# lipku/LiveTalking

Hardware: NVIDIA H100
Metric: lip-sync frames/sec (wav2lip256, 256x256, batch 16, mel + U-Net fwd + paste-back) (higher is better)
Workload: dtype f16 (fp32 accumulate); mel f64; paste u8

## Files before the change

### livetalking_b200/csrc/conv_gather.cu

```cuda
#include "conv_params.h"
#include "ltb_internal.h"
#include "ptx_sm90.cuh"

namespace ltb {

constexpr int kGatherThreads = 256;

template <int BN, int KB>
struct GatherCfg {
  static constexpr int CH = KB / 8;
  static constexpr int ROWB = KB * 2;
  static constexpr int RSTEP = kGatherThreads / CH;
  static constexpr int RPT = 128 / RSTEP;
  static constexpr int A_BYTES = 128 * ROWB;
  static constexpr int B_BYTES = (BN * ROWB < 1024) ? 1024 : BN * ROWB;
  static constexpr int STAGE_BYTES = A_BYTES + B_BYTES;
  static constexpr int STAGES = (STAGE_BYTES >= 32768) ? 3 : 4;
  static constexpr uint32_t LAYOUT = (KB == 64) ? 1u : (KB == 32) ? 2u : 3u;
  static constexpr uint32_t SBO = 8 * ROWB;
  static constexpr int SMEM_BYTES = STAGES * STAGE_BYTES + 1024;
};

template <int KB>
__device__ __forceinline__ uint32_t swz_chunk(int row, int j) {
  if (KB == 64) return (uint32_t)(j ^ (row & 7));
  if (KB == 32) return (uint32_t)(j ^ ((row >> 1) & 3));
  return (uint32_t)(j ^ ((row >> 2) & 1));
}

template <int BN, int KB, bool GRP>
__global__ void __launch_bounds__(kGatherThreads) conv_gather_wgmma_kernel(const __grid_constant__ ConvParams p) {
  using C = GatherCfg<BN, KB>;
  extern __shared__ uint8_t smem_raw[];
  const int tid = threadIdx.x;
  const int wg = tid >> 7, wq = (tid >> 5) & 3, lane = tid & 31;
  const uint32_t tiles = (smem_u32(smem_raw) + 1023u) & ~1023u;

  const int zphase = (p.ksplit > 1) ? 0 : ((p.zbatch > 1) ? (int)(blockIdx.z % p.nphases) : (int)blockIdx.z);
  const ConvPhase& ph = p.ph[zphase];
  const __half* in_base = p.in;
  const __half* w_base = p.w;
  __half* out_base = p.out;
  if (p.zbatch > 1) {
    const int zb = blockIdx.z / p.nphases;
    const int zo = zb / p.zdiv, zi = zb - zo * p.zdiv;
    in_base += zo * p.in_zo + zi * p.in_zi;
    w_base += zo * p.w_zo + zi * p.w_zi;
    out_base += zo * p.out_zo + zi * p.out_zi;
  }
  const int g_rows = GRP ? p.group_images * p.GH * p.GW : 0, g_tiles = (g_rows + 127) / 128;
  const int group = GRP ? (int)blockIdx.x / g_tiles : 0;
  const int m0 = GRP ? group * g_rows + ((int)blockIdx.x - group * g_tiles) * 128 : blockIdx.x * 128;
  const int n0 = blockIdx.y * BN;
  const int cpt = p.Cin / KB;
  int it_begin = 0, kiters = ph.ntaps * cpt;
  if (p.ksplit > 1) {
    const int per = (kiters + p.ksplit - 1) / p.ksplit;
    it_begin = (int)blockIdx.z * per;
    kiters = min(per, kiters - it_begin);
  }
  pdl_launch_dependents();
  pdl_wait();
  const float* bias_g = nullptr;
  if constexpr (GRP) {
    const int slot = p.group_slot[group];
    w_base += slot * p.w_slot_stride;
    bias_g = p.bias + slot * p.bias_slot_stride;
  }
  const float* const bias = GRP ? bias_g : p.bias;
  const int M = GRP ? (group + 1) * g_rows : p.M;

  const int j = tid % C::CH;
  const int r0 = tid / C::CH;
  int riy[C::RPT], rix[C::RPT];
  long long rbase[C::RPT];
  const int gsz = p.GH * p.GW;
#pragma unroll
  for (int i = 0; i < C::RPT; ++i) {
    const int m = m0 + r0 + i * C::RSTEP;
    if (m < M) {
      const int b = m / gsz;
      const int rem = m - b * gsz;
      const int gy = rem / p.GW;
      const int gx = rem - gy * p.GW;
      riy[i] = gy * p.sy;
      rix[i] = gx * p.sx;
      rbase[i] = ((long long)(b * p.IH + riy[i]) * p.IW + rix[i]) * p.ICtot + p.ic_off + j * 8;
    } else {
      riy[i] = -(1 << 20);
      rix[i] = 0;
      rbase[i] = 0;
    }
  }
  auto load = [&](int it) {
    const int kk = it_begin + it;
    const int tap = kk / cpt, cc = kk - tap * cpt;
    const uint32_t a_base = tiles + (it % C::STAGES) * C::STAGE_BYTES;
    const uint32_t b_base = a_base + C::A_BYTES;
    const int dy = ph.dy[tap], dx = ph.dx[tap];
    const long long toff = (long long)(dy * p.IW + dx) * p.ICtot + cc * KB;
#pragma unroll
    for (int i = 0; i < C::RPT; ++i) {
      const int row = r0 + i * C::RSTEP;
      const int iy = riy[i] + dy, ix = rix[i] + dx;
      const bool inb = ((unsigned)iy < (unsigned)p.IH) && ((unsigned)ix < (unsigned)p.IW);
      const __half* src = inb ? (in_base + rbase[i] + toff) : in_base;
      cp_async16(a_base + row * C::ROWB + swz_chunk<KB>(row, j) * 16, src, inb ? 16u : 0u);
    }
    const size_t wk = (size_t)ph.koff + (size_t)tap * p.Cin + cc * KB + j * 8;
#pragma unroll
    for (int i = 0; i < C::RPT; ++i) {
      const int n = r0 + i * C::RSTEP;
      if (n < BN) cp_async16(b_base + n * C::ROWB + swz_chunk<KB>(n, j) * 16, w_base + (size_t)(n0 + n) * p.Ktot + wk, 16u);
    }
  };

  float acc[BN / 2];
#pragma unroll
  for (int i = 0; i < BN / 2; ++i) acc[i] = 0.f;
#pragma unroll
  for (int s = 0; s < C::STAGES - 1; ++s) {
    if (s < kiters) load(s);
    cp_async_commit();
  }
  for (int it = 0; it < kiters; ++it) {
    cp_async_wait<C::STAGES - 2>();
    fence_proxy_async_smem();
    __syncthreads();
    if (it + C::STAGES - 1 < kiters) load(it + C::STAGES - 1);
    cp_async_commit();
    const uint32_t a_base = tiles + (it % C::STAGES) * C::STAGE_BYTES;
    const uint32_t b_base = a_base + C::A_BYTES;
    wgmma_fence();
#pragma unroll
    for (int k = 0; k < KB / 16; ++k) {
      const uint64_t ad = wgmma_desc(a_base + wg * 64 * C::ROWB + k * 32, 16, C::SBO, C::LAYOUT);
      const uint64_t bd = wgmma_desc(b_base + k * 32, 16, C::SBO, C::LAYOUT);
      Wgmma<BN>::ss(acc, ad, bd, 1u);
    }
    wgmma_commit();
    wgmma_wait<0>();
    wgmma_fence_regs(acc);
  }
  cp_async_wait<0>();

  const int cq = 2 * (lane & 3);
#pragma unroll
  for (int hh = 0; hh < 2; ++hh) {
    const int m = m0 + wg * 64 + wq * 16 + (lane >> 2) + 8 * hh;
    if (m >= M) continue;
    if (p.ksplit > 1) {
      float* wrow = p.ws + ((size_t)blockIdx.z * p.M + m) * p.Cout + n0;
#pragma unroll
      for (int i = 0; i < BN / 8; ++i)
        *reinterpret_cast<float2*>(wrow + 8 * i + cq) = make_float2(acc[4 * i + 2 * hh], acc[4 * i + 2 * hh + 1]);
      continue;
    }
    const int b = m / gsz;
    const int rem = m - b * gsz;
    const int gy = rem / p.GW;
    const int gx = rem - gy * p.GW;
    const size_t opix = (size_t)(b * p.OH + gy * p.osy + ph.ooy) * p.OW + gx * p.osx + ph.oox;
    __half* optr = out_base + opix * p.OCtot + p.oc_off + n0;
    const __half* rptr = p.res ? (p.res + opix * p.RCtot + p.rc_off + n0) : nullptr;
#pragma unroll
    for (int i = 0; i < BN / 8; ++i) {
      const int c = 8 * i + cq;
      const float2 bb = __ldg(reinterpret_cast<const float2*>(bias + n0 + c));
      float x = acc[4 * i + 2 * hh] + bb.x, y = acc[4 * i + 2 * hh + 1] + bb.y;
      if (rptr) {
        const float2 rf = __half22float2(__ldcg(reinterpret_cast<const __half2*>(rptr + c)));
        x += rf.x;
        y += rf.y;
      }
      if (p.relu) {
        x = fmaxf(x, 0.f);
        y = fmaxf(y, 0.f);
      }
      x = fminf(fmaxf(x, -65504.f), 65504.f);
      y = fminf(fmaxf(y, -65504.f), 65504.f);
      *reinterpret_cast<__half2*>(optr + c) = __floats2half2_rn(x, y);
    }
  }
}

template <int BN, int KB, bool GRP>
static cudaError_t launch_grp(const ConvParams& p, cudaStream_t st) {
  using C = GatherCfg<BN, KB>;
  static SmemConfigOnce once;
  if (cudaError_t e = once.ensure(conv_gather_wgmma_kernel<BN, KB, GRP>, C::SMEM_BYTES); e != cudaSuccess) return e;
  const int mt = GRP ? (p.N / p.group_images) * ((p.group_images * p.GH * p.GW + 127) / 128) : (p.M + 127) / 128;
  dim3 grid(mt, p.Cout / BN, p.ksplit > 1 ? p.ksplit : p.nphases * (p.zbatch > 1 ? p.zbatch : 1));
  return launch_kernel_pdl(conv_gather_wgmma_kernel<BN, KB, GRP>, grid, dim3(kGatherThreads), C::SMEM_BYTES, st, p);
}

template <int BN, int KB>
static cudaError_t launch_one(const ConvParams& p, cudaStream_t st) {
  return p.group_slot ? launch_grp<BN, KB, true>(p, st) : launch_grp<BN, KB, false>(p, st);
}

template <int KB>
static cudaError_t launch_kb(const ConvParams& p, int bn, cudaStream_t st) {
  switch (bn) {
    case 128: return launch_one<128, KB>(p, st);
    case 64: return launch_one<64, KB>(p, st);
    case 32: return launch_one<32, KB>(p, st);
    case 16: return launch_one<16, KB>(p, st);
  }
  return cudaErrorInvalidValue;
}

static int conv_gather_pick_bn(const ConvParams& p) {
  int bn = 0;
  for (int c : {128, 64, 32, 16})
    if (p.Cout % c == 0) {
      bn = c;
      break;
    }
  if (!bn) return 0;
  const long mt = (p.M + 127) / 128;
  const long zb = p.zbatch > 1 ? p.zbatch : 1;
  while (bn > 32 && mt * (p.Cout / bn) * p.nphases * zb < 132) bn >>= 1;
  return bn;
}

__global__ void __launch_bounds__(256) splitk_finalize_kernel(const float* __restrict__ ws, int ksplit, int M, int Cout,
                                                              const float* __restrict__ bias, const __half* __restrict__ res, int RCtot,
                                                              int rc_off, int relu, __half* __restrict__ out, int OCtot, int oc_off) {
  const unsigned vpr = Cout / 8;
  const unsigned total = (unsigned)M * vpr;
  const size_t slice = (size_t)M * Cout;
  pdl_launch_dependents();
  pdl_wait();
  for (unsigned i = blockIdx.x * 256u + threadIdx.x; i < total; i += gridDim.x * 256u) {
    const size_t m = i / vpr;
    const int c = (int)(i % vpr) * 8;
    float f[8];
#pragma unroll
    for (int j = 0; j < 8; ++j) f[j] = __ldg(bias + c + j);
    for (int s = 0; s < ksplit; ++s) {
      const float4* w4 = reinterpret_cast<const float4*>(ws + s * slice + m * Cout + c);
      const float4 a = __ldcg(w4), b = __ldcg(w4 + 1);
      f[0] += a.x; f[1] += a.y; f[2] += a.z; f[3] += a.w;
      f[4] += b.x; f[5] += b.y; f[6] += b.z; f[7] += b.w;
    }
    if (res) {
      const uint4 rv = __ldcg(reinterpret_cast<const uint4*>(res + m * RCtot + rc_off + c));
      const __half* rh = reinterpret_cast<const __half*>(&rv);
#pragma unroll
      for (int j = 0; j < 8; ++j) f[j] += __half2float(rh[j]);
    }
    uint4 ov;
    __half* oh = reinterpret_cast<__half*>(&ov);
#pragma unroll
    for (int j = 0; j < 8; ++j) {
      float x = relu ? fmaxf(f[j], 0.f) : f[j];
      oh[j] = __float2half_rn(fminf(fmaxf(x, -65504.f), 65504.f));
    }
    *reinterpret_cast<uint4*>(out + m * OCtot + oc_off + c) = ov;
  }
}

bool conv_gather_pick(const ConvParams& p, bool have_ws, size_t splitk_ws_floats, int* bn_out, int* kb_out, int* ksplit_out) {
  if (p.Cout % 16 != 0 || p.Cin % 16 != 0 || (p.ICtot % 8) || (p.OCtot % 8) || (p.ic_off % 8) || (p.oc_off % 8) ||
      (p.Ktot % 8) || p.nphases < 1 || p.nphases > kMaxPhases)
    return false;
  if (p.res && ((p.RCtot % 8) || (p.rc_off % 8))) return false;
  int bn = conv_gather_pick_bn(p);
  if (!bn) return false;
  const int kb = (p.Cin % 64 == 0) ? 64 : (p.Cin % 32 == 0) ? 32 : 16;
  int ksplit = 0;
  const int kiters = p.ph[0].ntaps * (p.Cin / kb);
  const long mt = (p.M + 127) / 128;
  if (have_ws && !p.group_slot && p.nphases == 1 && p.zbatch <= 1 && p.osy == 1 && p.osx == 1 && p.GH == p.OH && p.GW == p.OW && kiters >= 32 && mt <= 8) {
    int bn2 = 0;
    for (int c : {128, 64, 32, 16})
      if (p.Cout % c == 0) {
        bn2 = c;
        break;
      }
    const long tiles = mt * (p.Cout / bn2);
    if (tiles < 64) {
      int ks = (int)((264 + tiles - 1) / tiles);
      if (ks > kiters / 8) ks = kiters / 8;
      if (ks > 32) ks = 32;
      while (ks >= 2 && (size_t)ks * p.M * p.Cout > splitk_ws_floats) --ks;
      if (ks >= 2) {
        const int per = (kiters + ks - 1) / ks;
        ksplit = (kiters + per - 1) / per;
        bn = bn2;
      }
    }
  }
  *bn_out = bn;
  *kb_out = kb;
  *ksplit_out = ksplit;
  return true;
}

cudaError_t launch_conv_gather(const ConvParams& p_in, cudaStream_t st, float* splitk_ws, size_t splitk_ws_floats) {
  ConvParams p = p_in;
  int bn, kb;
  if (!conv_gather_pick(p, splitk_ws != nullptr, splitk_ws_floats, &bn, &kb, &p.ksplit)) return cudaErrorInvalidValue;
  p.ws = p.ksplit > 1 ? splitk_ws : nullptr;
  cudaError_t e;
  if (kb == 64) e = launch_kb<64>(p, bn, st);
  else if (kb == 32) e = launch_kb<32>(p, bn, st);
  else e = launch_kb<16>(p, bn, st);
  if (e != cudaSuccess || p.ksplit <= 1) return e;
  const size_t total = (size_t)p.M * (p.Cout / 8);
  int blocks = (int)((total + 255) / 256);
  if (blocks > 592) blocks = 592;
  return launch_kernel_pdl(splitk_finalize_kernel, dim3(blocks), dim3(256), 0, st, (const float*)p.ws, p.ksplit, p.M, p.Cout, p.bias, p.res,
                           p.RCtot, p.rc_off, p.relu, p.out, p.OCtot, p.oc_off);
}

}
```

### livetalking_b200/csrc/conv_plan.cu

```cuda
#include <cstring>
#include <string>
#include <vector>

#include "../../include/ltb200.h"
#include "conv_plan.h"
#include "ltb_internal.h"

namespace ltb {

static const int kTd[2][2] = {{0, 0}, {0, 1}};
static const int kTk[2][2] = {{1, 0}, {2, 0}};
static const int kTn[2] = {1, 2};
static const int kUd[2][2] = {{-1, 0}, {0, 1}};

ConvParams conv_params(ConvMode mode, int N, ConvSlice in, int IH, int IW, int Cin, ConvSlice out, int OH, int OW, int Cout,
                       ConvSlice res, const __half* w, int Ktot, int w_koff, const float* bias, bool relu, ConvTaps taps) {
  ConvParams p;
  std::memset(&p, 0, sizeof(p));
  p.in = in.p;
  p.N = N;
  p.IH = IH;
  p.IW = IW;
  p.ICtot = in.Ctot;
  p.ic_off = in.off;
  p.Cin = Cin;
  p.sy = p.sx = 1;
  p.out = const_cast<__half*>(out.p);
  p.OH = OH;
  p.OW = OW;
  p.OCtot = out.Ctot;
  p.oc_off = out.off;
  p.osy = p.osx = 1;
  p.Cout = Cout;
  p.res = res.p;
  p.RCtot = res.Ctot;
  p.rc_off = res.off;
  p.w = w;
  p.Ktot = Ktot;
  p.bias = bias;
  p.relu = relu ? 1 : 0;
  if (mode == ConvMode::Dense) {
    p.sy = taps.sy;
    p.sx = taps.sx;
    p.GH = OH;
    p.GW = OW;
    p.nphases = 1;
    ConvPhase& ph = p.ph[0];
    ph.ntaps = taps.KH * taps.KW;
    ph.koff = w_koff;
    for (int kh = 0; kh < taps.KH; ++kh)
      for (int kw = 0; kw < taps.KW; ++kw) {
        ph.dy[kh * taps.KW + kw] = (signed char)(kh - taps.pad_t);
        ph.dx[kh * taps.KW + kw] = (signed char)(kw - taps.pad_l);
      }
  } else {
    const bool up = mode == ConvMode::Upsample2x;
    p.GH = IH;
    p.GW = IW;
    p.osy = p.osx = 2;
    p.nphases = 4;
    p.upconv = up ? 1 : 0;
    int koff = w_koff;
    for (int a = 0; a < 2; ++a)
      for (int b = 0; b < 2; ++b) {
        ConvPhase& ph = p.ph[a * 2 + b];
        const int na = up ? 2 : kTn[a], nb = up ? 2 : kTn[b];
        ph.ntaps = na * nb;
        ph.koff = koff;
        ph.ooy = a;
        ph.oox = b;
        for (int i = 0; i < na; ++i)
          for (int j = 0; j < nb; ++j) {
            ph.dy[i * nb + j] = (signed char)(up ? kUd[a][i] : kTd[a][i]);
            ph.dx[i * nb + j] = (signed char)(up ? kUd[b][j] : kTd[b][j]);
          }
        koff += ph.ntaps * Cin;
      }
  }
  p.M = N * p.GH * p.GW;
  return p;
}

int conv_plan(const ConvParams& p, const __half* w_tap, ConvPath path, ConvPlan* out) {
  out->p = p;
  out->halo = false;
  if (p.group_slot) {
    if (p.group_images < 1 || p.N % p.group_images || p.slots < 1 || p.w_slot_stride < 0 || p.bias_slot_stride < 0)
      return LTB_FAIL("conv: grouped weights need N divisible by group_images >= 1, slots >= 1 and non-negative slot strides");
    if (p.zbatch > 1 || p.upconv) return LTB_FAIL("conv: grouped weights cannot be combined with zbatch or the fused upsample");
  }
  if (path == ConvPath::Gather) return 0;
  const bool gemm = p.nphases == 1 && p.ph[0].ntaps == 1;
  if (!((w_tap || gemm) && conv_halo_supported(p))) {
    if (path == ConvPath::Auto) return 0;
    return LTB_FAIL("conv: the halo kernel cannot run " + std::to_string(p.N) + "x" + std::to_string(p.IH) + "x" + std::to_string(p.IW) +
                    "x" + std::to_string(p.Cin) + " -> " + std::to_string(p.OH) + "x" + std::to_string(p.OW) + "x" + std::to_string(p.Cout) +
                    (w_tap || gemm ? "" : " without tap-major weights"));
  }
  if (conv_halo_make_plan(p, w_tap, &out->hp) != 0) return LTB_FAIL("conv: halo plan / tensor map creation failed");
  out->halo = true;
  return 0;
}

cudaError_t conv_launch(const ConvPlan& pl, cudaStream_t st, float* splitk_ws, size_t ws_floats) {
  return pl.halo ? launch_conv_halo(pl.hp, st) : launch_conv_gather(pl.p, st, splitk_ws, ws_floats);
}

bool conv_plan_variant(const ConvPlan& pl, bool have_ws, size_t ws_floats, ltb_conv_variant* out) {
  std::memset(out, 0, sizeof(*out));
  out->grouped = pl.p.group_slot != nullptr;
  if (pl.halo) {
    out->kernel = 1;
    out->taps = pl.hp.TAPS;
    out->bn = pl.hp.BN;
    out->nsub = pl.hp.NSUB;
    out->nacc = pl.hp.NACC;
    out->resident_chunks = conv_halo_resident_chunks(pl.hp, conv_halo_sms());
    out->res_halo = pl.hp.hp.res_halo;
    return true;
  }
  int ksplit = 0;
  if (!conv_gather_pick(pl.p, have_ws, ws_floats, &out->bn, &out->kb, &ksplit)) return false;
  out->ksplit = ksplit > 1 ? ksplit : 1;
  return true;
}

bool conv_plan_fuse_gn_stats(ConvPlan* pl, float* stats, int groups, int hw) {
  const ConvParams& p = pl->p;
  if (!pl->halo || pl->hp.grouped || p.oc_off != 0 || p.OCtot != p.Cout || !conv_halo_gn_fusable(pl->hp, p.Cout, groups, hw)) return false;
  HaloParams& h = pl->hp.hp;
  h.gn_stats = stats;
  h.gn_groups = groups;
  h.gn_cpg = p.Cout / groups;
  h.gn_hw = hw;
  h.gn_images = p.M / hw;
  return true;
}

bool conv_plan_fuse_head(ConvPlan* pl, const float* w, const float* b, float* out) {
  if (!pl->halo || pl->hp.grouped || pl->hp.BN != 32 || pl->p.Cout != 32) return false;
  pl->hp.hp.head_w = w;
  pl->hp.hp.head_b = b;
  pl->hp.hp.head_out = out;
  return true;
}

static void pack_conv_w(const float* w, int cout, int cin, int KH, int KW, std::vector<__half>& out) {
  out.resize((size_t)cout * KH * KW * cin);
  for (int co = 0; co < cout; ++co)
    for (int kh = 0; kh < KH; ++kh)
      for (int kw = 0; kw < KW; ++kw)
        for (int ci = 0; ci < cin; ++ci)
          out[((size_t)co * KH * KW + kh * KW + kw) * cin + ci] = __float2half(w[(((size_t)co * cin + ci) * KH + kh) * KW + kw]);
}
static void pack_convT_w(const float* w, int cin, int cout, std::vector<__half>& out) {
  out.resize((size_t)cout * 9 * cin);
  for (int co = 0; co < cout; ++co) {
    size_t k = 0;
    for (int a = 0; a < 2; ++a)
      for (int b = 0; b < 2; ++b)
        for (int i = 0; i < kTn[a]; ++i)
          for (int j = 0; j < kTn[b]; ++j) {
            const int kh = kTk[a][i], kw = kTk[b][j];
            for (int ci = 0; ci < cin; ++ci, ++k)
              out[(size_t)co * 9 * cin + k] = __float2half(w[(((size_t)ci * cout + co) * 3 + kh) * 3 + kw]);
          }
  }
}

}

using namespace ltb;

static int conv2d_f16_impl(const ltb_conv_desc* d, const void* in_f16, const float* w_f32, const float* bias_f32,
                           const void* res_f16, void* out_f16, int reps, float* ms_out) {
  if (!d || !in_f16 || !w_f32 || !bias_f32 || !out_f16) return LTB_FAIL("null argument");
  if (d->has_res && !res_f16) return LTB_FAIL("has_res set but res is null");
  int OH, OW, Ktot;
  std::vector<__half> wp;
  if (d->transposed) {
    if (d->KH != 3 || d->KW != 3) return LTB_FAIL("transposed conv: only k=3,s=2,p=1,op=1");
    OH = d->IH * 2;
    OW = d->IW * 2;
    Ktot = 9 * d->Cin;
    pack_convT_w(w_f32, d->Cin, d->Cout, wp);
  } else {
    if (d->KH * d->KW > kMaxTaps) return LTB_FAIL("kernel too large");
    OH = conv_out_dim(d->IH, d->KH, d->sy, d->pad);
    OW = conv_out_dim(d->IW, d->KW, d->sx, d->pad);
    Ktot = d->KH * d->KW * d->Cin;
    pack_conv_w(w_f32, d->Cout, d->Cin, d->KH, d->KW, wp);
  }
  if (OH <= 0 || OW <= 0) return LTB_FAIL("empty output");
  const size_t in_b = (size_t)d->N * d->IH * d->IW * d->Cin * 2, out_b = (size_t)d->N * OH * OW * d->Cout * 2;
  __half *din = nullptr, *dout = nullptr, *dw = nullptr, *dres = nullptr, *dwt = nullptr;
  float* dbias = nullptr;
  float* dws = nullptr;
  cudaEvent_t e0 = nullptr, e1 = nullptr;
  int rc = 0;
  auto cleanup = [&]() {
    cudaFree(din);
    cudaFree(dout);
    cudaFree(dw);
    cudaFree(dres);
    cudaFree(dwt);
    cudaFree(dws);
    cudaFree(dbias);
    if (e0) cudaEventDestroy(e0);
    if (e1) cudaEventDestroy(e1);
  };
#define CK(x)                                                             \
  do {                                                                    \
    cudaError_t _e = (x);                                                 \
    if (_e != cudaSuccess) {                                              \
      rc = LTB_FAIL(std::string(#x) + ": " + cudaGetErrorString(_e));     \
      cleanup();                                                          \
      return rc;                                                          \
    }                                                                     \
  } while (0)
  CK(cudaMalloc(&din, in_b));
  CK(cudaMalloc(&dout, out_b));
  CK(cudaMalloc(&dw, wp.size() * 2));
  CK(cudaMalloc(&dbias, (size_t)d->Cout * 4));
  CK(cudaMemcpy(din, in_f16, in_b, cudaMemcpyHostToDevice));
  CK(cudaMemcpy(dw, wp.data(), wp.size() * 2, cudaMemcpyHostToDevice));
  CK(cudaMemcpy(dbias, bias_f32, (size_t)d->Cout * 4, cudaMemcpyHostToDevice));
  CK(cudaMemset(dout, 0xFF, out_b));
  if (d->has_res) {
    CK(cudaMalloc(&dres, out_b));
    CK(cudaMemcpy(dres, res_f16, out_b, cudaMemcpyHostToDevice));
  }
  if (d->KH == 3 && d->KW == 3) {
    CK(cudaMalloc(&dwt, wp.size() * 2));
    CK(d->transposed ? launch_w_tap_major_convT(dw, dwt, d->Cout, d->Cin, nullptr) : launch_w_tap_major(dw, dwt, d->Cout, d->Cin, nullptr));
  }
  const ConvParams p = conv_params(d->transposed ? ConvMode::Transposed : ConvMode::Dense, d->N, {din, d->Cin, 0}, d->IH, d->IW, d->Cin,
                                   {dout, d->Cout, 0}, OH, OW, d->Cout, d->has_res ? ConvSlice{dres, d->Cout, 0} : ConvSlice{}, dw, Ktot, 0,
                                   dbias, d->relu != 0, {d->KH, d->KW, d->sy, d->sx, d->pad, d->pad});
  const ConvPath path = d->force_path == 1 ? ConvPath::Gather : d->force_path == 2 ? ConvPath::Halo : ConvPath::Auto;
  ConvPlan pl;
  if (conv_plan(p, dwt, path, &pl)) {
    cleanup();
    return 1;
  }
  const size_t ws_floats = pl.halo ? 0 : (size_t)1 << 22;
  if (ws_floats) {
    CK(cudaMalloc(&dws, ws_floats * sizeof(float)));
    CK(cudaMemset(dws, 0, ws_floats * sizeof(float)));
  }
  CK(conv_launch(pl, nullptr, dws, ws_floats));
  if (reps > 0) {
    CK(cudaEventCreate(&e0));
    CK(cudaEventCreate(&e1));
    for (int i = 0; i < 3; ++i) CK(conv_launch(pl, nullptr, dws, ws_floats));
    CK(cudaEventRecord(e0, nullptr));
    for (int i = 0; i < reps; ++i) CK(conv_launch(pl, nullptr, dws, ws_floats));
    CK(cudaEventRecord(e1, nullptr));
    CK(cudaEventSynchronize(e1));
    CK(cudaEventElapsedTime(ms_out, e0, e1));
    *ms_out /= reps;
  }
  CK(cudaDeviceSynchronize());
  CK(cudaMemcpy(out_f16, dout, out_b, cudaMemcpyDeviceToHost));
#undef CK
  cleanup();
  return 0;
}

extern "C" {

int ltb_conv2d_f16(const ltb_conv_desc* d, const void* in_f16, const float* w_f32, const float* bias_f32,
                   const void* res_f16, void* out_f16) {
  return conv2d_f16_impl(d, in_f16, w_f32, bias_f32, res_f16, out_f16, 0, nullptr);
}

int ltb_conv2d_f16_timed(const ltb_conv_desc* d, const void* in_f16, const float* w_f32, const float* bias_f32,
                         const void* res_f16, void* out_f16, int reps, float* ms_per_launch) {
  if (reps < 1 || !ms_per_launch) return LTB_FAIL("conv2d_f16_timed: reps >= 1 and a result pointer are required");
  return conv2d_f16_impl(d, in_f16, w_f32, bias_f32, res_f16, out_f16, reps, ms_per_launch);
}

}
```

Baseline: 6889.

## Extend split-K to transposed-conv phases and 1x1 row GEMMs; route small convs to gather

Generalizes the split-K gather path so the grid z-dimension covers phases times k-splits, letting the 4-phase transposed convolutions and tiny 1x1 spatial GEMMs split their reduction across more CTAs. The finalize kernel now takes the full params and maps each phase's rows back to strided output pixels for residual and output writes. Small-spatial 3x3 and transposed convs (<=4x4) skip the halo kernel and use the gather/split-K path by default. This targets under-filled SMs on the low-resolution U-Net layers, at the cost of an fp32 workspace round trip and an extra finalize launch.

```diff
diff --git a/livetalking_b200/csrc/conv_gather.cu b/livetalking_b200/csrc/conv_gather.cu
--- a/livetalking_b200/csrc/conv_gather.cu
+++ b/livetalking_b200/csrc/conv_gather.cu
@@ -1,3 +1,5 @@
+#include <algorithm>
+
 #include "conv_params.h"
 #include "ltb_internal.h"
 #include "ptx_sm90.cuh"
@@ -36,7 +38,7 @@
   const int wg = tid >> 7, wq = (tid >> 5) & 3, lane = tid & 31;
   const uint32_t tiles = (smem_u32(smem_raw) + 1023u) & ~1023u;
 
-  const int zphase = (p.ksplit > 1) ? 0 : ((p.zbatch > 1) ? (int)(blockIdx.z % p.nphases) : (int)blockIdx.z);
+  const int zphase = (p.ksplit > 1) ? (int)blockIdx.z / p.ksplit : ((p.zbatch > 1) ? (int)(blockIdx.z % p.nphases) : (int)blockIdx.z);
   const ConvPhase& ph = p.ph[zphase];
   const __half* in_base = p.in;
   const __half* w_base = p.w;
@@ -56,7 +58,7 @@
   int it_begin = 0, kiters = ph.ntaps * cpt;
   if (p.ksplit > 1) {
     const int per = (kiters + p.ksplit - 1) / p.ksplit;
-    it_begin = (int)blockIdx.z * per;
+    it_begin = ((int)blockIdx.z - zphase * p.ksplit) * per;
     kiters = min(per, kiters - it_begin);
   }
   pdl_launch_dependents();
@@ -190,7 +192,7 @@
   static SmemConfigOnce once;
   if (cudaError_t e = once.ensure(conv_gather_wgmma_kernel<BN, KB, GRP>, C::SMEM_BYTES); e != cudaSuccess) return e;
   const int mt = GRP ? (p.N / p.group_images) * ((p.group_images * p.GH * p.GW + 127) / 128) : (p.M + 127) / 128;
-  dim3 grid(mt, p.Cout / BN, p.ksplit > 1 ? p.ksplit : p.nphases * (p.zbatch > 1 ? p.zbatch : 1));
+  dim3 grid(mt, p.Cout / BN, p.nphases * (p.ksplit > 1 ? p.ksplit : (p.zbatch > 1 ? p.zbatch : 1)));
   return launch_kernel_pdl(conv_gather_wgmma_kernel<BN, KB, GRP>, grid, dim3(kGatherThreads), C::SMEM_BYTES, st, p);
 }
 
@@ -224,28 +226,37 @@
   return bn;
 }
 
-__global__ void __launch_bounds__(256) splitk_finalize_kernel(const float* __restrict__ ws, int ksplit, int M, int Cout,
-                                                              const float* __restrict__ bias, const __half* __restrict__ res, int RCtot,
-                                                              int rc_off, int relu, __half* __restrict__ out, int OCtot, int oc_off) {
-  const unsigned vpr = Cout / 8;
-  const unsigned total = (unsigned)M * vpr;
-  const size_t slice = (size_t)M * Cout;
+__global__ void __launch_bounds__(256) splitk_finalize_kernel(const __grid_constant__ ConvParams p) {
+  const unsigned vpr = p.Cout / 8;
+  const unsigned per_phase = (unsigned)p.M * vpr;
+  const unsigned total = per_phase * p.nphases;
+  const size_t slice = (size_t)p.M * p.Cout;
+  const int gsz = p.GH * p.GW;
   pdl_launch_dependents();
   pdl_wait();
   for (unsigned i = blockIdx.x * 256u + threadIdx.x; i < total; i += gridDim.x * 256u) {
-    const size_t m = i / vpr;
-    const int c = (int)(i % vpr) * 8;
+    const int phase = (int)(i / per_phase);
+    const unsigned e = i - phase * per_phase;
+    const int m = (int)(e / vpr);
+    const int c = (int)(e % vpr) * 8;
     float f[8];
 #pragma unroll
-    for (int j = 0; j < 8; ++j) f[j] = __ldg(bias + c + j);
-    for (int s = 0; s < ksplit; ++s) {
-      const float4* w4 = reinterpret_cast<const float4*>(ws + s * slice + m * Cout + c);
+    for (int j = 0; j < 8; ++j) f[j] = __ldg(p.bias + c + j);
+    const float* wsp = p.ws + (size_t)phase * p.ksplit * slice + (size_t)m * p.Cout + c;
+    for (int s = 0; s < p.ksplit; ++s) {
+      const float4* w4 = reinterpret_cast<const float4*>(wsp + s * slice);
       const float4 a = __ldcg(w4), b = __ldcg(w4 + 1);
       f[0] += a.x; f[1] += a.y; f[2] += a.z; f[3] += a.w;
       f[4] += b.x; f[5] += b.y; f[6] += b.z; f[7] += b.w;
     }
-    if (res) {
-      const uint4 rv = __ldcg(reinterpret_cast<const uint4*>(res + m * RCtot + rc_off + c));
+    const ConvPhase& ph = p.ph[phase];
+    const int b = m / gsz;
+    const int rem = m - b * gsz;
+    const int gy = rem / p.GW;
+    const int gx = rem - gy * p.GW;
+    const size_t opix = (size_t)(b * p.OH + gy * p.osy + ph.ooy) * p.OW + gx * p.osx + ph.oox;
+    if (p.res) {
+      const uint4 rv = __ldcg(reinterpret_cast<const uint4*>(p.res + opix * p.RCtot + p.rc_off + c));
       const __half* rh = reinterpret_cast<const __half*>(&rv);
 #pragma unroll
       for (int j = 0; j < 8; ++j) f[j] += __half2float(rh[j]);
@@ -254,10 +265,10 @@
     __half* oh = reinterpret_cast<__half*>(&ov);
 #pragma unroll
     for (int j = 0; j < 8; ++j) {
-      float x = relu ? fmaxf(f[j], 0.f) : f[j];
+      float x = p.relu ? fmaxf(f[j], 0.f) : f[j];
       oh[j] = __float2half_rn(fminf(fmaxf(x, -65504.f), 65504.f));
     }
-    *reinterpret_cast<uint4*>(out + m * OCtot + oc_off + c) = ov;
+    *reinterpret_cast<uint4*>(p.out + opix * p.OCtot + p.oc_off + c) = ov;
   }
 }
 
@@ -270,24 +281,36 @@
   if (!bn) return false;
   const int kb = (p.Cin % 64 == 0) ? 64 : (p.Cin % 32 == 0) ? 32 : 16;
   int ksplit = 0;
-  const int kiters = p.ph[0].ntaps * (p.Cin / kb);
+  const bool convt = p.nphases == 4 && !p.upconv && p.osy == 2 && p.osx == 2;
+  int kiters = 0, kmin = 1 << 30;
+  for (int i = 0; i < p.nphases; ++i) {
+    kiters = std::max(kiters, p.ph[i].ntaps * (p.Cin / kb));
+    kmin = std::min(kmin, p.ph[i].ntaps * (p.Cin / kb));
+  }
   const long mt = (p.M + 127) / 128;
-  if (have_ws && !p.group_slot && p.nphases == 1 && p.zbatch <= 1 && p.osy == 1 && p.osx == 1 && p.GH == p.OH && p.GW == p.OW && kiters >= 32 && mt <= 8) {
+  const bool dense = p.nphases == 1 && p.osy == 1 && p.osx == 1 && p.GH == p.OH && p.GW == p.OW;
+  const bool row = dense && p.ph[0].ntaps == 1 && p.GH == 1 && p.GW == 1 && kiters >= 8;
+  if (have_ws && !p.group_slot && p.zbatch <= 1 && (dense || convt) && (kiters >= 32 || row) && mt <= 8) {
     int bn2 = 0;
     for (int c : {128, 64, 32, 16})
       if (p.Cout % c == 0) {
         bn2 = c;
         break;
       }
-    const long tiles = mt * (p.Cout / bn2);
-    if (tiles < 64) {
+    const long tiles = mt * (p.Cout / bn2) * p.nphases;
+    const bool wide = dense && kiters >= 32 && tiles < 64;
+    if (wide || (convt && tiles < 264) || (row && tiles < 132)) {
       int ks = (int)((264 + tiles - 1) / tiles);
-      if (ks > kiters / 8) ks = kiters / 8;
+      const int per_min = (wide || convt) ? 8 : 2;
+      if (ks > kiters / per_min) ks = kiters / per_min;
+      if (ks > kiters * kb / 128) ks = kiters * kb / 128;
       if (ks > 32) ks = 32;
-      while (ks >= 2 && (size_t)ks * p.M * p.Cout > splitk_ws_floats) --ks;
+      while (ks >= 2 && (size_t)ks * p.nphases * p.M * p.Cout > splitk_ws_floats) --ks;
+      if (convt)
+        while (ks >= 2 && (ks - 1) * ((kmin + ks - 1) / ks) >= kmin) --ks;
       if (ks >= 2) {
         const int per = (kiters + ks - 1) / ks;
-        ksplit = (kiters + per - 1) / per;
+        ksplit = convt ? ks : (kiters + per - 1) / per;
         bn = bn2;
       }
     }
@@ -308,11 +331,10 @@
   else if (kb == 32) e = launch_kb<32>(p, bn, st);
   else e = launch_kb<16>(p, bn, st);
   if (e != cudaSuccess || p.ksplit <= 1) return e;
-  const size_t total = (size_t)p.M * (p.Cout / 8);
+  const size_t total = (size_t)p.nphases * p.M * (p.Cout / 8);
   int blocks = (int)((total + 255) / 256);
   if (blocks > 592) blocks = 592;
-  return launch_kernel_pdl(splitk_finalize_kernel, dim3(blocks), dim3(256), 0, st, (const float*)p.ws, p.ksplit, p.M, p.Cout, p.bias, p.res,
-                           p.RCtot, p.rc_off, p.relu, p.out, p.OCtot, p.oc_off);
-}
-
-}
+  return launch_kernel_pdl(splitk_finalize_kernel, dim3(blocks), dim3(256), 0, st, p);
+}
+
+}
diff --git a/livetalking_b200/csrc/conv_plan.cu b/livetalking_b200/csrc/conv_plan.cu
--- a/livetalking_b200/csrc/conv_plan.cu
+++ b/livetalking_b200/csrc/conv_plan.cu
@@ -90,6 +90,9 @@
     if (p.zbatch > 1 || p.upconv) return LTB_FAIL("conv: grouped weights cannot be combined with zbatch or the fused upsample");
   }
   if (path == ConvPath::Gather) return 0;
+  const bool conv3x3 = p.nphases == 1 && p.ph[0].ntaps == 9 && p.sy == 1 && p.sx == 1;
+  const bool convT = p.nphases == 4 && !p.upconv;
+  if (path == ConvPath::Auto && !p.group_slot && ((conv3x3 && p.GH <= 4 && p.GW <= 4) || (convT && p.GH <= 4 && p.GW <= 4))) return 0;
   const bool gemm = p.nphases == 1 && p.ph[0].ntaps == 1;
   if (!((w_tap || gemm) && conv_halo_supported(p))) {
     if (path == ConvPath::Auto) return 0;
@@ -243,7 +246,7 @@
     cleanup();
     return 1;
   }
-  const size_t ws_floats = pl.halo ? 0 : (size_t)1 << 22;
+  const size_t ws_floats = pl.halo ? 0 : (size_t)8 << 20;
   if (ws_floats) {
     CK(cudaMalloc(&dws, ws_floats * sizeof(float)));
     CK(cudaMemset(dws, 0, ws_floats * sizeof(float)));
```

Result: no change. 6992 (median of 6 runs) (+1.5%).
